# uc-vision/smart-tree

Hardware: AMD Instinct MI355X
Metric: points/sec end-to-end (voxelize->sparse-UNet->skeleton), 1M-pt tree (higher is better)
Workload: dtype f32

## Files before the change

smart_tree_amd/csrc/graph.hip:

```cpp
#include "st_common.h"
#include "st_grid.h"

#define GR_BLOCK 256
static inline unsigned gr_grid(int64_t n) {
    int64_t g = st_div_up(n > 0 ? n : 1, GR_BLOCK);
    return (unsigned)(g < 8192 ? g : 8192);
}
#define GR_LOOP(i, n) for (int64_t i = (int64_t)blockIdx.x * blockDim.x + threadIdx.x; i < (n); i += (int64_t)gridDim.x * blockDim.x)

__global__ void __launch_bounds__(GR_BLOCK) k_medial(const float* xyz, const float* mv, int64_t n, float* medial, float* radius) {
    GR_LOOP(i, n) {
        const float x = mv[3 * i], y = mv[3 * i + 1], z = mv[3 * i + 2];
        medial[3 * i] = xyz[3 * i] + x;
        medial[3 * i + 1] = xyz[3 * i + 1] + y;
        medial[3 * i + 2] = xyz[3 * i + 2] + z;
        float s = x * x;
        float t = y * y;
        s = s + t;
        t = z * z;
        s = s + t;
        radius[i] = sqrtf(s);
    }
}

extern "C" int st_medial_points(const float* xyz, const float* mv, int64_t n, float* medial, float* radius, void* stream_) {
    if (n <= 0) return ST_OK;
    hipLaunchKernelGGL(k_medial, dim3(gr_grid(n)), dim3(GR_BLOCK), 0, (hipStream_t)stream_, xyz, mv, n, medial, radius);
    ST_CHECK_LAUNCH();
    return ST_OK;
}

struct GrRange {
    int64_t i0, i1;
    int64_t a0, a1;
    int64_t nq;
};
__device__ __forceinline__ GrRange gr_range(const void* p0, const void* p1, int64_t n, const int* seg_off, int seg) {
    GrRange r;
    r.i0 = seg_off ? seg_off[seg] : 0;
    r.i1 = seg_off ? seg_off[seg + 1] : n;
    const bool vec = ((((uintptr_t)p0) | ((uintptr_t)p1)) & 15) == 0;
    r.a0 = vec ? st_min((r.i0 + 3) & ~(int64_t)3, r.i1) : r.i1;
    r.a1 = r.a0 + ((r.i1 - r.a0) & ~(int64_t)3);
    r.nq = (r.a1 - r.a0) / 4 * 3;
    return r;
}
__device__ __forceinline__ int64_t gr_edge_point(const GrRange& r, int64_t j) { return j < r.a0 - r.i0 ? r.i0 + j : r.a1 + (j - (r.a0 - r.i0)); }

__global__ void __launch_bounds__(GR_BLOCK) k_bbox(const float* xyz, int64_t n, unsigned* box, const int* seg_off) {
    __shared__ unsigned lo[3], hi[3];
    if (threadIdx.x < 3) { lo[threadIdx.x] = 0xffffffffu; hi[threadIdx.x] = 0u; }
    __syncthreads();
    const int seg = blockIdx.y;
    const GrRange r = gr_range(xyz, nullptr, n, seg_off, seg);
    unsigned lx = 0xffffffffu, ly = 0xffffffffu, lz = 0xffffffffu, hx = 0u, hy = 0u, hz = 0u;
    const float4* v = reinterpret_cast<const float4*>(xyz + 3 * r.a0);
    for (int64_t q = (int64_t)blockIdx.x * blockDim.x + threadIdx.x; q < r.nq; q += (int64_t)gridDim.x * blockDim.x) {
        const float4 f = v[q];
        const int ax = (int)(q % 3);
        const unsigned o0 = st_f2ord(f.x), o1 = st_f2ord(f.y), o2 = st_f2ord(f.z), o3 = st_f2ord(f.w);
        const unsigned a = st_min(o0, o3), b = st_max(o0, o3);
        lx = st_min(lx, ax == 0 ? a : (ax == 1 ? o2 : o1)); hx = st_max(hx, ax == 0 ? b : (ax == 1 ? o2 : o1));
        ly = st_min(ly, ax == 0 ? o1 : (ax == 1 ? a : o2)); hy = st_max(hy, ax == 0 ? o1 : (ax == 1 ? b : o2));
        lz = st_min(lz, ax == 0 ? o2 : (ax == 1 ? o1 : a)); hz = st_max(hz, ax == 0 ? o2 : (ax == 1 ? o1 : b));
    }
    const int64_t ne = (r.a0 - r.i0) + (r.i1 - r.a1);
    for (int64_t j = (int64_t)blockIdx.x * blockDim.x + threadIdx.x; j < ne; j += (int64_t)gridDim.x * blockDim.x) {
        const int64_t i = gr_edge_point(r, j);
        const unsigned ox = st_f2ord(xyz[3 * i]), oy = st_f2ord(xyz[3 * i + 1]), oz = st_f2ord(xyz[3 * i + 2]);
        lx = st_min(lx, ox); hx = st_max(hx, ox); ly = st_min(ly, oy); hy = st_max(hy, oy); lz = st_min(lz, oz); hz = st_max(hz, oz);
    }
    for (int d = 32; d > 0; d >>= 1) {
        lx = st_min(lx, (unsigned)__shfl_xor((int)lx, d)); ly = st_min(ly, (unsigned)__shfl_xor((int)ly, d)); lz = st_min(lz, (unsigned)__shfl_xor((int)lz, d));
        hx = st_max(hx, (unsigned)__shfl_xor((int)hx, d)); hy = st_max(hy, (unsigned)__shfl_xor((int)hy, d)); hz = st_max(hz, (unsigned)__shfl_xor((int)hz, d));
    }
    if ((threadIdx.x & 63) == 0) {
        atomicMin(&lo[0], lx); atomicMin(&lo[1], ly); atomicMin(&lo[2], lz);
        atomicMax(&hi[0], hx); atomicMax(&hi[1], hy); atomicMax(&hi[2], hz);
    }
    __syncthreads();
    if (threadIdx.x < 3 && r.i1 > r.i0) { atomicMin(&box[6 * seg + threadIdx.x], lo[threadIdx.x]); atomicMax(&box[6 * seg + 3 + threadIdx.x], hi[threadIdx.x]); }
}
__global__ void __launch_bounds__(GR_BLOCK) k_centre(const float* xyz, int64_t n, const unsigned* box, float* out, const int* seg_off,
                                                     float* box_out) {
    const int seg = blockIdx.y;
    const GrRange r = gr_range(xyz, out, n, seg_off, seg);
    float shift[3];
    for (int a = 0; a < 3; a++) {
        const float mn = st_ord2f(box[6 * seg + a]), mx = st_ord2f(box[6 * seg + 3 + a]);
        const float half = (mx - mn) / 2.0f;
        const float centre = mn + half;
        shift[a] = -centre + (a == 1 ? half : 0.0f);
        if (box_out && blockIdx.x == 0 && threadIdx.x == 0) {
            box_out[6 * seg + a] = r.i1 > r.i0 ? mn + shift[a] : INFINITY;
            box_out[6 * seg + 3 + a] = r.i1 > r.i0 ? mx + shift[a] : -INFINITY;
        }
    }
    const float4* v = reinterpret_cast<const float4*>(xyz + 3 * r.a0);
    float4* o = reinterpret_cast<float4*>(out + 3 * r.a0);
    for (int64_t q = (int64_t)blockIdx.x * blockDim.x + threadIdx.x; q < r.nq; q += (int64_t)gridDim.x * blockDim.x) {
        float4 f = v[q];
        const int ax = (int)(q % 3);
        const float s0 = ax == 0 ? shift[0] : (ax == 1 ? shift[1] : shift[2]);
        const float s1 = ax == 0 ? shift[1] : (ax == 1 ? shift[2] : shift[0]);
        const float s2 = ax == 0 ? shift[2] : (ax == 1 ? shift[0] : shift[1]);
        f.x = f.x + s0; f.y = f.y + s1; f.z = f.z + s2; f.w = f.w + s0;
        o[q] = f;
    }
    const int64_t ne = (r.a0 - r.i0) + (r.i1 - r.a1);
    for (int64_t j = (int64_t)blockIdx.x * blockDim.x + threadIdx.x; j < ne; j += (int64_t)gridDim.x * blockDim.x) {
        const int64_t i = gr_edge_point(r, j);
        for (int a = 0; a < 3; a++) out[3 * i + a] = xyz[3 * i + a] + shift[a];
    }
}

__global__ void k_box_init(unsigned* box, int nseg) {
    for (int i = threadIdx.x; i < 6 * nseg; i += blockDim.x) box[i] = i % 6 < 3 ? 0xffffffffu : 0u;
}

extern "C" int st_centre_cloud_box_seg(const float* xyz, int64_t n, const int32_t* seg_off, int nseg, float* out, void* ws,
                                       int64_t ws_bytes, void* stream_, float* box_out) {
    hipStream_t stream = (hipStream_t)stream_;
    if (n <= 0) {
        ST_REQUIRE(!box_out, "centre_cloud: no box of an empty array");
        return ST_OK;
    }
    ST_REQUIRE(nseg >= 1 && nseg <= ST_MAX_SEG && (nseg == 1 || seg_off), "centre_cloud: 1 <= clouds per batch <= %d", ST_MAX_SEG);
    if (nseg == 1) seg_off = nullptr;
    StArena a(ws, ws_bytes);
    unsigned* box = a.take<unsigned>(6 * (int64_t)nseg);
    if (!box) { st_set_error("centre_cloud: workspace too small"); return ST_ERR_WORKSPACE; }
    hipLaunchKernelGGL(k_box_init, dim3(1), dim3(64), 0, stream, box, nseg);
    const int64_t per = st_div_up(st_div_up(3 * n, 4), nseg);
    const unsigned gx = (unsigned)st_min64(st_div_up(per > 0 ? per : 1, GR_BLOCK), 2048 / (nseg < 8 ? nseg : 8) + 1);
    hipLaunchKernelGGL(k_bbox, dim3(gx, (unsigned)nseg), dim3(GR_BLOCK), 0, stream, xyz, n, box, seg_off);
    hipLaunchKernelGGL(k_centre, dim3((unsigned)st_min64(st_div_up(per > 0 ? per : 1, GR_BLOCK), 8192), (unsigned)nseg), dim3(GR_BLOCK), 0, stream,
                       xyz, n, (const unsigned*)box, out, seg_off, box_out);
    ST_CHECK_LAUNCH();
    return ST_OK;
}
extern "C" int st_centre_cloud_seg(const float* xyz, int64_t n, const int32_t* seg_off, int nseg, float* out, void* ws,
                                   int64_t ws_bytes, void* stream_) {
    return st_centre_cloud_box_seg(xyz, n, seg_off, nseg, out, ws, ws_bytes, stream_, nullptr);
}
extern "C" int st_centre_cloud(const float* xyz, int64_t n, float* out, void* ws, int64_t ws_bytes, void* stream_) {
    return st_centre_cloud_seg(xyz, n, nullptr, 1, out, ws, ws_bytes, stream_);
}

__global__ void __launch_bounds__(GR_BLOCK) k_edge_count(const int64_t* idx, int64_t n, int K, uint32_t* cnt, const int* seg_off,
                                                         int nseg) {
    GR_LOOP(i, n) {
        const int64_t first = seg_off ? seg_off[st_seg_find(seg_off, nseg, i)] : 0;
        uint32_t c = 0;
        for (int k = 0; k < K; k++) c += idx[i * K + k] > first;
        cnt[i] = c;
    }
}
__global__ void __launch_bounds__(GR_BLOCK) k_edge_emit(const int64_t* idx, const float* dist, int64_t n, int K,
                                                        const uint32_t* off, int64_t* edges, float* w, const int* seg_off,
                                                        int nseg) {
    GR_LOOP(i, n) {
        const int64_t first = seg_off ? seg_off[st_seg_find(seg_off, nseg, i)] : 0;
        uint32_t o = off[i];
        for (int k = 0; k < K; k++) {
            int64_t j = idx[i * K + k];
            if (j > first) { edges[2 * (int64_t)o] = i; edges[2 * (int64_t)o + 1] = j; w[o] = dist[i * K + k]; o++; }
        }
    }
}

extern "C" int64_t st_make_edges_workspace_bytes(int64_t n) {
    StArena a(nullptr, 0);
    a.take<uint32_t>(n + 1);
    a.take<char>(st_scan_ws_bytes(n));
    return a.used;
}

__global__ void __launch_bounds__(GR_BLOCK) k_edge_pad(int64_t* edges, float* w, const uint32_t* total, int64_t cap) {
    for (int64_t e = (int64_t)*total + (int64_t)blockIdx.x * blockDim.x + threadIdx.x; e < cap; e += (int64_t)gridDim.x * blockDim.x) {
        edges[2 * e] = 0;
        edges[2 * e + 1] = 0;
        w[e] = 0.0f;
    }
}

extern "C" int st_make_edges_seg(const int64_t* idx, const float* dist, int64_t n, int K, int64_t* edges, float* w,
                                 int64_t* n_edges_host, const int32_t* seg_off, int nseg, void* ws, int64_t ws_bytes,
                                 void* stream_) {
    hipStream_t stream = (hipStream_t)stream_;
    if (n_edges_host) *n_edges_host = 0;
    if (n <= 0) return ST_OK;
    ST_REQUIRE(nseg >= 1 && nseg <= ST_MAX_SEG && (nseg == 1 || seg_off), "make_edges: 1 <= clouds per batch <= %d", ST_MAX_SEG);
    if (nseg == 1) seg_off = nullptr;
    StArena a(ws, ws_bytes);
    uint32_t* cnt = a.take<uint32_t>(n + 1);
    int64_t sb = st_scan_ws_bytes(n);
    char* sw = a.take<char>(sb);
    if (!cnt || !sw) { st_set_error("make_edges: workspace too small"); return ST_ERR_WORKSPACE; }
    hipLaunchKernelGGL(k_edge_count, dim3(gr_grid(n)), dim3(GR_BLOCK), 0, stream, idx, n, K, cnt, seg_off, nseg);
    ST_TRY(st_exclusive_scan_u32(cnt, cnt, n, cnt + n, sw, sb, stream));
    hipLaunchKernelGGL(k_edge_emit, dim3(gr_grid(n)), dim3(GR_BLOCK), 0, stream, idx, dist, n, K, (const uint32_t*)cnt, edges, w,
                       seg_off, nseg);
    if (!n_edges_host) {
        hipLaunchKernelGGL(k_edge_pad, dim3(64), dim3(GR_BLOCK), 0, stream, edges, w, (const uint32_t*)(cnt + n), n * (int64_t)K);
        ST_CHECK_LAUNCH();
        return ST_OK;
    }
    uint32_t total = 0;
    (void)hipMemcpyAsync(&total, cnt + n, sizeof(uint32_t), hipMemcpyDeviceToHost, stream);
    st_stream_wait(stream);
    ST_CHECK_LAUNCH();
    *n_edges_host = total;
    return ST_OK;
}

extern "C" int st_make_edges(const int64_t* idx, const float* dist, int64_t n, int K, int64_t* edges, float* w,
                             int64_t* n_edges_host, void* ws, int64_t ws_bytes, void* stream_) {
    return st_make_edges_seg(idx, dist, n, K, edges, w, n_edges_host, nullptr, 1, ws, ws_bytes, stream_);
}

struct GrEdges {
    const int64_t* edges;
    const float* w;
    const int64_t* idx;
    const float* dist;
    int K, k_shift;
    const int* first_of;
};
static inline int gr_shift_of(int K) { int sh = 0; while ((1 << sh) < K) sh++; return (1 << sh) == K ? sh : -1; }
__device__ __forceinline__ void gr_edge(const GrEdges& G, int64_t e, int64_t* u, int64_t* v) {
    if (G.idx == nullptr) { *u = G.edges[2 * e]; *v = G.edges[2 * e + 1]; return; }
    const int64_t i = G.k_shift >= 0 ? (e >> G.k_shift) : e / G.K, j = G.idx[e];
    const int64_t first = G.first_of ? G.first_of[i] : 0;
    *u = i;
    *v = j > first ? j : i;
}
__device__ __forceinline__ float gr_edge_weight(const GrEdges& G, int64_t e) { return G.idx ? G.dist[e] : G.w[e]; }

#define CC_MUL 0x9E3779B1u
#define CC_INV 0x0E8B2F51u
__device__ __forceinline__ unsigned cc_key(unsigned x) { return x * CC_MUL; }
__device__ __forceinline__ unsigned cc_idx(unsigned k) { return k * CC_INV; }

__device__ __forceinline__ unsigned cc_find(unsigned* label, unsigned k) {
    unsigned p = __atomic_load_n(&label[cc_idx(k)], __ATOMIC_RELAXED);
    while (p != k) {
        const unsigned gp = __atomic_load_n(&label[cc_idx(p)], __ATOMIC_RELAXED);
        if (gp != p) atomicMin(&label[cc_idx(k)], gp);
        k = p;
        p = gp;
    }
    return k;
}
__global__ void __launch_bounds__(GR_BLOCK) k_cc_init(unsigned* label, int64_t n) { GR_LOOP(i, n) label[i] = cc_key((unsigned)i); }
__global__ void __launch_bounds__(GR_BLOCK) k_cc_hook(GrEdges G, int64_t E, unsigned* label, int sample) {
    GR_LOOP(e, E) {
        if (sample && (((uint32_t)e * 2654435761u) >> 29) != 0u) continue;
        int64_t u64, v64;
        gr_edge(G, e, &u64, &v64);
        const unsigned u = (unsigned)u64, v = (unsigned)v64;
        if (u == v) continue;
        if (!sample) {
            if (label[u] == label[v]) continue;
        }
        unsigned a = cc_find(label, cc_key(u)), b = cc_find(label, cc_key(v));
        while (a != b) {
            if (a < b) { const unsigned t = a; a = b; b = t; }
            const unsigned seen = atomicCAS(&label[cc_idx(a)], a, b);
            if (seen == a) break;
            a = seen;
        }
    }
}
__global__ void __launch_bounds__(GR_BLOCK) k_cc_compress(unsigned* label, int64_t n) {
    GR_LOOP(i, n) { const unsigned r = cc_find(label, cc_key((unsigned)i)); label[i] = r; }
}
__global__ void __launch_bounds__(GR_BLOCK) k_cc_minid_init(unsigned* minid, int64_t n) { GR_LOOP(i, n) minid[i] = 0xffffffffu; }
__global__ void __launch_bounds__(GR_BLOCK) k_cc_minid(const unsigned* label, int64_t n, unsigned* minid) {
    const int lane = threadIdx.x & 63;
    for (int64_t base = (int64_t)blockIdx.x * blockDim.x; base < n; base += (int64_t)gridDim.x * blockDim.x) {
        const int64_t i = base + threadIdx.x;
        const bool valid = i < n;
        const unsigned r = valid ? cc_idx(label[i]) : 0xffffffffu;
        unsigned long long todo = __ballot(valid);
        while (todo) {
            const int leader = __ffsll(todo) - 1;
            const unsigned lr = __shfl(r, leader);
            const unsigned long long same = __ballot(valid && r == lr);
            if (lane == leader) atomicMin(&minid[lr], (unsigned)i);
            todo &= ~same;
        }
    }
}
__global__ void __launch_bounds__(GR_BLOCK) k_cc_relabel(unsigned* label, int64_t n, const unsigned* minid) {
    GR_LOOP(i, n) label[i] = minid[cc_idx(label[i])];
}

extern "C" int64_t st_connected_components_workspace_bytes(int64_t n) { return (n > 0 ? n : 1) * (int64_t)sizeof(unsigned) + 256; }

static int cc_run(GrEdges G, int64_t E, int64_t n, int32_t* labels, void* ws, int64_t ws_bytes, void* stream_);

extern "C" int st_connected_components(const int64_t* edges, int64_t E, int64_t n, int32_t* labels, void* ws,
                                       int64_t ws_bytes, void* stream_) {
    GrEdges G = {edges, nullptr, nullptr, nullptr, 0, -1, nullptr};
    return cc_run(G, E, n, labels, ws, ws_bytes, stream_);
}

extern "C" int st_connected_components_knn(const int64_t* idx, int64_t n, int K, const int32_t* first_of,
                                           int32_t* labels, void* ws, int64_t ws_bytes, void* stream_) {
    ST_REQUIRE(K >= 1, "cc(knn): K must be positive");
    GrEdges G = {nullptr, nullptr, idx, nullptr, K, gr_shift_of(K), first_of};
    return cc_run(G, n * (int64_t)K, n, labels, ws, ws_bytes, stream_);
}

static int cc_run(GrEdges G, int64_t E, int64_t n, int32_t* labels, void* ws, int64_t ws_bytes, void* stream_) {
    hipStream_t stream = (hipStream_t)stream_;
    ST_REQUIRE(n < (1ll << 31), "cc: too many vertices");
    if (n <= 0) return ST_OK;
    StArena ar(ws, ws_bytes);
    unsigned* minid = ar.take<unsigned>(n);
    if (!ar.ok() || !minid) {
        st_set_error("cc: workspace too small (%lld < %lld)", (long long)ws_bytes, (long long)ar.used);
        return ST_ERR_WORKSPACE;
    }
    unsigned* label = (unsigned*)labels;
    hipLaunchKernelGGL(k_cc_init, dim3(gr_grid(n)), dim3(GR_BLOCK), 0, stream, label, n);
    if (E > 0) {
        hipLaunchKernelGGL(k_cc_hook, dim3(gr_grid(E)), dim3(GR_BLOCK), 0, stream, G, E, label, 1);
        hipLaunchKernelGGL(k_cc_compress, dim3(gr_grid(n)), dim3(GR_BLOCK), 0, stream, label, n);
        hipLaunchKernelGGL(k_cc_hook, dim3(gr_grid(E)), dim3(GR_BLOCK), 0, stream, G, E, label, 0);
    }
    hipLaunchKernelGGL(k_cc_compress, dim3(gr_grid(n)), dim3(GR_BLOCK), 0, stream, label, n);
    hipLaunchKernelGGL(k_cc_minid_init, dim3(gr_grid(n)), dim3(GR_BLOCK), 0, stream, minid, n);
    hipLaunchKernelGGL(k_cc_minid, dim3(gr_grid(n)), dim3(GR_BLOCK), 0, stream, (const unsigned*)label, n, minid);
    hipLaunchKernelGGL(k_cc_relabel, dim3(gr_grid(n)), dim3(GR_BLOCK), 0, stream, label, n, (const unsigned*)minid);
    ST_CHECK_LAUNCH();
    return ST_OK;
}

__global__ void __launch_bounds__(GR_BLOCK) k_cl_sizes(const int* label, int64_t n, uint32_t* size) {
    const int lane = threadIdx.x & 63;
    for (int64_t base = (int64_t)blockIdx.x * blockDim.x; base < n; base += (int64_t)gridDim.x * blockDim.x) {
        const int64_t i = base + threadIdx.x;
        const bool valid = i < n;
        const int lab = valid ? label[i] : -1;
        unsigned long long todo = __ballot(valid);
        while (todo) {
            const int leader = __ffsll(todo) - 1;
            const int l = __shfl(lab, leader);
            const unsigned long long same = __ballot(valid && lab == l);
            if (lane == leader) atomicAdd(&size[l], (uint32_t)__popcll(same));
            todo &= ~same;
        }
    }
}
__global__ void __launch_bounds__(GR_BLOCK) k_cl_rootflag(const int* label, const uint32_t* size, int64_t n, uint32_t minv,
                                                          uint32_t* flag, uint32_t* kept) {
    GR_LOOP(i, n) {
        const bool root = label[i] == (int)i && size[i] >= minv;
        flag[i] = root ? 1u : 0u;
        if (root) { atomicAdd(kept, size[i]); atomicMax(kept + 1, size[i]); }
    }
}
__global__ void __launch_bounds__(GR_BLOCK) k_cl_rootlist(const uint32_t* flag_off, const int* label, const uint32_t* size,
                                                          int64_t n, uint32_t minv, uint32_t* key, uint32_t* root) {
    GR_LOOP(i, n) if (label[i] == (int)i && size[i] >= minv) { key[flag_off[i]] = 0xffffffffu - size[i]; root[flag_off[i]] = (uint32_t)i; }
}
__global__ void __launch_bounds__(GR_BLOCK) k_cl_rank(const uint32_t* root_sorted, const uint32_t* size, int64_t C,
                                                      int* rank_of_root, uint32_t* comp_size) {
    GR_LOOP(c, C) { rank_of_root[root_sorted[c]] = (int)c; comp_size[c] = size[root_sorted[c]]; }
}
__global__ void __launch_bounds__(GR_BLOCK) k_cl_segkey(const uint32_t* root_sorted, int64_t C, const int* seg_off, int nseg,
                                                        uint32_t* key) {
    GR_LOOP(c, C) key[c] = (uint32_t)st_seg_find(seg_off, nseg, root_sorted[c]);
}
__global__ void __launch_bounds__(GR_BLOCK) k_cl_segments(const uint32_t* root_sorted, int C, const int* seg_off, int nseg,
                                                          const int32_t* comp_off, int32_t* comp_seg, int32_t* comp_seg_off,
                                                          int32_t* vert_seg_off) {
    for (int b = threadIdx.x; b <= nseg; b += blockDim.x) comp_seg_off[b] = C;
    __syncthreads();
    for (int c = threadIdx.x; c < C; c += blockDim.x) {
        const int s = st_seg_find(seg_off, nseg, root_sorted[c]);
        comp_seg[c] = s;
        const int prev = c > 0 ? st_seg_find(seg_off, nseg, root_sorted[c - 1]) : -1;
        for (int b = prev + 1; b <= s; b++) comp_seg_off[b] = c;
    }
    __syncthreads();
    for (int b = threadIdx.x; b <= nseg; b += blockDim.x) vert_seg_off[b] = comp_off[comp_seg_off[b]];
}
__global__ void __launch_bounds__(GR_BLOCK) k_cl_vflag(const int* label, const int* rank_of_root, int64_t n, uint32_t* flag) {
    GR_LOOP(i, n) flag[i] = rank_of_root[label[i]] >= 0 ? 1u : 0u;
}
__global__ void __launch_bounds__(GR_BLOCK) k_cl_vlist(const uint32_t* flag_off, const int* label, const int* rank_of_root,
                                                       int64_t n, uint32_t* vkey, uint32_t* vid) {
    GR_LOOP(i, n) {
        int r = rank_of_root[label[i]];
        if (r >= 0) { vkey[flag_off[i]] = (uint32_t)r; vid[flag_off[i]] = (uint32_t)i; }
    }
}
__global__ void __launch_bounds__(GR_BLOCK) k_cl_newid(const uint32_t* vid_sorted, int64_t m, int* new_id, int32_t* vert_order) {
    GR_LOOP(p, m) { new_id[vid_sorted[p]] = (int)p; vert_order[p] = (int32_t)vid_sorted[p]; }
}
__global__ void __launch_bounds__(GR_BLOCK) k_fill_i32(int* p, int64_t n, int v) { GR_LOOP(i, n) p[i] = v; }

extern "C" int64_t st_component_layout_workspace_bytes(int64_t n) {
    StArena a(nullptr, 0);
    a.take<uint32_t>(n + 2);
    a.take<uint32_t>(n + 1);
    a.take<uint32_t>(n);
    a.take<uint32_t>(n);
    a.take<int>(n);
    a.take<char>(st_sort_ws_bytes(n) > st_scan_ws_bytes(n + 1) ? st_sort_ws_bytes(n) : st_scan_ws_bytes(n + 1));
    return a.used;
}

extern "C" int st_component_layout_seg(const int32_t* labels, int64_t n, int min_vertices, const int32_t* seg_off, int nseg,
                                       int32_t* comp_size, int32_t* comp_off, int32_t* vert_order, int32_t* new_id,
                                       int32_t* comp_seg, int32_t* comp_seg_off, int32_t* vert_seg_off,
                                       int64_t* n_comp_host, int64_t* n_kept_host, void* ws, int64_t ws_bytes, void* stream_,
                                       int64_t* max_comp_host ) {
    hipStream_t stream = (hipStream_t)stream_;
    *n_comp_host = 0;
    *n_kept_host = 0;
    if (max_comp_host) *max_comp_host = 0;
    ST_REQUIRE(nseg >= 1 && nseg <= ST_MAX_SEG, "component_layout: 1 <= clouds per batch <= %d", ST_MAX_SEG);
    ST_REQUIRE(nseg == 1 || (seg_off && comp_seg && comp_seg_off && vert_seg_off), "component_layout: a batch needs seg_off and the per-cloud outputs");
    if (n <= 0) {
        if (nseg > 1) { (void)hipMemsetAsync(comp_seg_off, 0, (nseg + 1) * sizeof(int32_t), stream); (void)hipMemsetAsync(vert_seg_off, 0, (nseg + 1) * sizeof(int32_t), stream); }
        return ST_OK;
    }
    StArena a(ws, ws_bytes);
    uint32_t* size = a.take<uint32_t>(n + 2);
    uint32_t* flag = a.take<uint32_t>(n + 1);
    uint32_t* key = a.take<uint32_t>(n);
    uint32_t* val = a.take<uint32_t>(n);
    int* rank_of_root = a.take<int>(n);
    int64_t sb = st_sort_ws_bytes(n) > st_scan_ws_bytes(n + 1) ? st_sort_ws_bytes(n) : st_scan_ws_bytes(n + 1);
    char* sw = a.take<char>(sb);
    if (!a.ok() || !sw) { st_set_error("component_layout: workspace too small"); return ST_ERR_WORKSPACE; }
    const unsigned g = gr_grid(n);
    uint32_t minv = min_vertices > 0 ? (uint32_t)min_vertices : 0u;
    (void)hipMemsetAsync(size, 0, (n + 2) * sizeof(uint32_t), stream);
    hipLaunchKernelGGL(k_cl_sizes, dim3(g), dim3(GR_BLOCK), 0, stream, labels, n, size);
    hipLaunchKernelGGL(k_cl_rootflag, dim3(g), dim3(GR_BLOCK), 0, stream, labels, (const uint32_t*)size, n, minv, flag, size + n);
    ST_TRY(st_exclusive_scan_u32(flag, flag, n, flag + n, sw, sb, stream));
    uint32_t C = 0, mk[2] = {0, 0};
    (void)hipMemcpyAsync(&C, flag + n, sizeof(uint32_t), hipMemcpyDeviceToHost, stream);
    (void)hipMemcpyAsync(mk, size + n, 2 * sizeof(uint32_t), hipMemcpyDeviceToHost, stream);
    st_stream_wait(stream);
    const uint32_t m = mk[0];
    if (max_comp_host) *max_comp_host = mk[1];
    ST_CHECK_LAUNCH();
    hipLaunchKernelGGL(k_fill_i32, dim3(g), dim3(GR_BLOCK), 0, stream, new_id, n, -1);
    if (C == 0) {
        (void)hipMemsetAsync(comp_off, 0, sizeof(int32_t), stream);
        if (nseg > 1) { (void)hipMemsetAsync(comp_seg_off, 0, (nseg + 1) * sizeof(int32_t), stream); (void)hipMemsetAsync(vert_seg_off, 0, (nseg + 1) * sizeof(int32_t), stream); }
        ST_CHECK_LAUNCH();
        return ST_OK;
    }
    hipLaunchKernelGGL(k_cl_rootlist, dim3(g), dim3(GR_BLOCK), 0, stream, (const uint32_t*)flag, labels, (const uint32_t*)size, n,
                       minv, key, val);
    ST_TRY(st_radix_sort_pairs_u32(key, val, C, 32, sw, sb, stream));
    if (nseg > 1) {
        int sbits = 1;
        while ((1 << sbits) < nseg) sbits++;
        hipLaunchKernelGGL(k_cl_segkey, dim3(gr_grid(C)), dim3(GR_BLOCK), 0, stream, (const uint32_t*)val, (int64_t)C, seg_off, nseg, key);
        ST_TRY(st_radix_sort_pairs_u32(key, val, C, sbits, sw, sb, stream));
    }
    hipLaunchKernelGGL(k_fill_i32, dim3(g), dim3(GR_BLOCK), 0, stream, rank_of_root, n, -1);
    hipLaunchKernelGGL(k_cl_rank, dim3(gr_grid(C)), dim3(GR_BLOCK), 0, stream, (const uint32_t*)val, (const uint32_t*)size,
                       (int64_t)C, rank_of_root, (uint32_t*)comp_size);
    ST_TRY(st_exclusive_scan_u32((const uint32_t*)comp_size, (uint32_t*)comp_off, C, (uint32_t*)comp_off + C, sw, sb, stream));
    if (nseg > 1)
        hipLaunchKernelGGL(k_cl_segments, dim3(1), dim3(GR_BLOCK), 0, stream, (const uint32_t*)val, (int)C, seg_off, nseg,
                           (const int32_t*)comp_off, comp_seg, comp_seg_off, vert_seg_off);
    hipLaunchKernelGGL(k_cl_vflag, dim3(g), dim3(GR_BLOCK), 0, stream, labels, (const int*)rank_of_root, n, flag);
    ST_TRY(st_exclusive_scan_u32(flag, flag, n, flag + n, sw, sb, stream));
    hipLaunchKernelGGL(k_cl_vlist, dim3(g), dim3(GR_BLOCK), 0, stream, (const uint32_t*)flag, labels, (const int*)rank_of_root, n,
                       key, val);
    int bits = 1;
    while ((1u << bits) < C && bits < 32) bits++;
    ST_TRY(st_radix_sort_pairs_u32(key, val, m, bits, sw, sb, stream));
    hipLaunchKernelGGL(k_cl_newid, dim3(gr_grid(m)), dim3(GR_BLOCK), 0, stream, (const uint32_t*)val, (int64_t)m, new_id,
                       vert_order);
    ST_CHECK_LAUNCH();
    *n_comp_host = C;
    *n_kept_host = m;
    return ST_OK;
}

extern "C" int st_component_layout(const int32_t* labels, int64_t n, int min_vertices, int32_t* comp_size, int32_t* comp_off,
                                   int32_t* vert_order, int32_t* new_id, int64_t* n_comp_host, int64_t* n_kept_host,
                                   void* ws, int64_t ws_bytes, void* stream_) {
    return st_component_layout_seg(labels, n, min_vertices, nullptr, 1, comp_size, comp_off, vert_order, new_id, nullptr, nullptr,
                                   nullptr, n_comp_host, n_kept_host, ws, ws_bytes, stream_, nullptr);
}

__device__ __forceinline__ uint32_t gr_run_add(uint32_t* ctr, int key) {
    const int lane = threadIdx.x & 63;
    const int prev = __shfl_up(key, 1);
    const bool head = key >= 0 && (lane == 0 || prev != key);
    const unsigned long long heads = __ballot(head), active = __ballot(key >= 0);
    const unsigned long long upto = heads & (~0ull >> (63 - lane));
    const int h = 63 - __clzll((long long)(upto | 1ull));
    const unsigned long long stop = (heads | ~active) & ~(~0ull >> (63 - h));
    const int end = stop ? __ffsll((long long)stop) - 1 : 64;
    uint32_t base = 0;
    if (head) base = atomicAdd(&ctr[key], (uint32_t)(end - lane));
    base = __shfl(base, h);
    return base + (uint32_t)(lane - h);
}

__device__ __forceinline__ void csr_edge_ends(const GrEdges& G, int64_t E, const int* new_id, int64_t e, int* a, int* b) {
    *a = -1; *b = -1;
    if (e >= E) return;
    int64_t u, v;
    gr_edge(G, e, &u, &v);
    if (u == v) return;
    const int x = new_id[u], y = new_id[v];
    if (x < 0 || y < 0) return;
    *a = x; *b = y;
}

__global__ void __launch_bounds__(GR_BLOCK) k_csr_count(GrEdges G, int64_t E, const int* new_id, uint32_t* deg) {
    const int lane = threadIdx.x & 63;
    for (int64_t base = (int64_t)blockIdx.x * blockDim.x + (threadIdx.x - lane); base < E; base += (int64_t)gridDim.x * blockDim.x) {
        int a, b;
        csr_edge_ends(G, E, new_id, base + lane, &a, &b);
        gr_run_add(deg, a);
        if (b >= 0) atomicAdd(&deg[b], 1u);
    }
}
__global__ void __launch_bounds__(GR_BLOCK) k_csr_fill(GrEdges G, int64_t E, const int* new_id,
                                                       uint32_t* cursor, uint32_t* col, float* wgt) {
    const int lane = threadIdx.x & 63;
    for (int64_t base = (int64_t)blockIdx.x * blockDim.x + (threadIdx.x - lane); base < E; base += (int64_t)gridDim.x * blockDim.x) {
        int a, b;
        csr_edge_ends(G, E, new_id, base + lane, &a, &b);
        const uint32_t pa = gr_run_add(cursor, a);
        if (a < 0) continue;
        const float we = gr_edge_weight(G, base + lane);
        col[pa] = (uint32_t)b; wgt[pa] = we;
        const uint32_t pb = atomicAdd(&cursor[b], 1u);
        col[pb] = (uint32_t)a; wgt[pb] = we;
    }
}

#define CSRK_MUTUAL 0x40000000
struct __attribute__((aligned(16))) GrI64x2 { int64_t x, y; };
struct __attribute__((aligned(16))) GrI32x4 { int32_t x, y, z, w; };
__global__ void __launch_bounds__(GR_BLOCK) k_csrk_pack(const int64_t* __restrict__ idx, int64_t E, int32_t* __restrict__ idx32) {
    GR_LOOP(e, E) idx32[e] = (int32_t)idx[e];
}
template <int K, bool PACKED>
__global__ void __launch_bounds__(GR_BLOCK) k_csrk_count(const int64_t* __restrict__ idx, const int32_t* __restrict__ idx32, int64_t n,
                                                         const int* __restrict__ first_of, const int* __restrict__ new_id, uint32_t* deg,
                                                         uint32_t* fwdc, int32_t* __restrict__ tgt) {
    const int64_t E = n * K;
    const int lane = threadIdx.x & 63;
    for (int64_t base = (int64_t)blockIdx.x * blockDim.x + (threadIdx.x - lane); base < E; base += (int64_t)gridDim.x * blockDim.x) {
        const int64_t e = base + lane;
        const int64_t i = e / K;
        int x = -1, y = -1;
        bool mutual = false;
        if (e < E) {
            x = new_id[i];
            const int64_t j = PACKED ? (int64_t)idx32[e] : idx[e], first = first_of ? first_of[i] : 0;
            if (x >= 0 && j > first && j != i) {
                y = new_id[j];
                if (y >= 0 && i > first) {
                    const int64_t* row = idx + j * K;
                    if (PACKED && K % 4 == 0) {
                        const int32_t* row32 = idx32 + j * K;
                        const int32_t i32 = (int32_t)i;
#pragma unroll
                        for (int k = 0; k < K; k += 4) {
                            const GrI32x4 r = *reinterpret_cast<const GrI32x4*>(row32 + k);
                            mutual = mutual || r.x == i32 || r.y == i32 || r.z == i32 || r.w == i32;
                        }
                    } else if (PACKED) {
                        for (int k = 0; k < K; k++) mutual = mutual || (int64_t)idx32[j * K + k] == i;
                    } else if (K % 2 == 0) {
#pragma unroll
                        for (int k = 0; k < K; k += 2) {
                            const GrI64x2 r = *reinterpret_cast<const GrI64x2*>(row + k);
                            mutual = mutual || r.x == i || r.y == i;
                        }
                    } else {
                        for (int k = 0; k < K; k++) mutual = mutual || row[k] == i;
                    }
                }
            }
        }
        const bool fwd = y >= 0;
        const unsigned long long fb = __ballot(fwd);
        if (e < E) tgt[e] = fwd ? (y | (mutual ? CSRK_MUTUAL : 0)) : -1;
        if (fwd && !mutual) atomicAdd(&deg[y], 1u);
        if ((lane % K) == 0 && x >= 0) {
            const unsigned cnt = (unsigned)__popcll(K == 64 ? fb : (fb >> lane) & ((1ull << (K & 63)) - 1ull));
            fwdc[x] = cnt;
            if (cnt) atomicAdd(&deg[x], cnt);
        }
    }
}
template <int K>
__global__ void __launch_bounds__(GR_BLOCK) k_csrk_fill(const int64_t n, const float* __restrict__ dist, const int* __restrict__ new_id,
                                                        const int32_t* __restrict__ tgt, const uint32_t* __restrict__ row_off,
                                                        uint32_t* cursor, uint32_t* __restrict__ col, float* __restrict__ wgt) {
    const int64_t E = n * K;
    const int lane = threadIdx.x & 63;
    for (int64_t base = (int64_t)blockIdx.x * blockDim.x + (threadIdx.x - lane); base < E; base += (int64_t)gridDim.x * blockDim.x) {
        const int64_t e = base + lane;
        const int32_t t = e < E ? tgt[e] : -1;
        const bool fwd = t >= 0;
        const unsigned long long fb = __ballot(fwd);
        if (!fwd) continue;
        const int x = new_id[e / K], y = t & ~CSRK_MUTUAL;
        const float we = dist[e];
        const int k = lane % K;
        const unsigned long long mine = K == 64 ? fb : (fb >> (lane - k)) & ((1ull << (K & 63)) - 1ull);
        const uint32_t pa = row_off[x] + (uint32_t)__popcll(mine & ((1ull << k) - 1ull));
        col[pa] = (uint32_t)y; wgt[pa] = we;
        if (!(t & CSRK_MUTUAL)) {
            const uint32_t pb = atomicAdd(&cursor[y], 1u);
            col[pb] = (uint32_t)x; wgt[pb] = we;
        }
    }
}
__global__ void __launch_bounds__(GR_BLOCK) k_csrk_cursor(const uint32_t* __restrict__ row_off, const uint32_t* __restrict__ fwdc, int64_t m,
                                                          uint32_t* __restrict__ cursor) {
    GR_LOOP(v, m) cursor[v] = row_off[v] + fwdc[v];
}

extern "C" int64_t st_component_csr_workspace_bytes(int64_t m) {
    StArena a(nullptr, 0);
    a.take<uint32_t>(m + 1);
    a.take<char>(st_scan_ws_bytes(m + 1));
    return a.used;
}
extern "C" int64_t st_component_csr_knn_workspace_bytes(int64_t m, int64_t n, int K) {
    StArena a(nullptr, 0);
    a.take<uint32_t>(m + 1);
    a.take<char>(st_scan_ws_bytes(m + 1));
    a.take<uint32_t>(m + 1);
    a.take<int32_t>(n * (int64_t)(K > 0 ? K : 1));
    a.take<int32_t>(n * (int64_t)(K > 0 ? K : 1));
    return a.used;
}

static int csr_run(GrEdges G, int64_t E, const int32_t* new_id, int64_t m, uint32_t* row_off, uint32_t* col, float* wgt, void* ws,
                   int64_t ws_bytes, void* stream_);

extern "C" int st_component_csr(const int64_t* edges, const float* w, int64_t E, const int32_t* new_id, int64_t m,
                                uint32_t* row_off, uint32_t* col, float* wgt, void* ws, int64_t ws_bytes, void* stream_) {
    GrEdges G = {edges, w, nullptr, nullptr, 0, -1, nullptr};
    return csr_run(G, E, new_id, m, row_off, col, wgt, ws, ws_bytes, stream_);
}

template <int K>
static void csrk_launch(const int64_t* idx, const float* dist, int64_t n, const int32_t* first_of, const int32_t* new_id, int64_t m,
                        uint32_t* row_off, uint32_t* col, float* wgt, uint32_t* cursor, uint32_t* fwdc, int32_t* tgt, int32_t* idx32,
                        char* sw, int64_t sb, hipStream_t stream, int* rc) {
    const int64_t E = n * K;
    (void)hipMemsetAsync(row_off, 0, (m + 1) * sizeof(uint32_t), stream);
    if (idx32) {
        hipLaunchKernelGGL(k_csrk_pack, dim3(gr_grid(E)), dim3(GR_BLOCK), 0, stream, idx, E, idx32);
        hipLaunchKernelGGL((k_csrk_count<K, true>), dim3(gr_grid(E)), dim3(GR_BLOCK), 0, stream, idx, (const int32_t*)idx32, n, first_of,
                           new_id, row_off, fwdc, tgt);
    } else {
        hipLaunchKernelGGL((k_csrk_count<K, false>), dim3(gr_grid(E)), dim3(GR_BLOCK), 0, stream, idx, (const int32_t*)nullptr, n, first_of,
                           new_id, row_off, fwdc, tgt);
    }
    *rc = st_exclusive_scan_u32(row_off, row_off, m + 1, nullptr, sw, sb, stream);
    if (*rc != ST_OK) return;
    hipLaunchKernelGGL(k_csrk_cursor, dim3(gr_grid(m)), dim3(GR_BLOCK), 0, stream, (const uint32_t*)row_off, (const uint32_t*)fwdc, m, cursor);
    hipLaunchKernelGGL((k_csrk_fill<K>), dim3(gr_grid(E)), dim3(GR_BLOCK), 0, stream, n, dist, new_id, (const int32_t*)tgt,
                       (const uint32_t*)row_off, cursor, col, wgt);
}
extern "C" int st_component_csr_knn(const int64_t* idx, const float* dist, int64_t n, int K, const int32_t* first_of,
                                    const int32_t* new_id, int64_t m, uint32_t* row_off, uint32_t* col, float* wgt, void* ws,
                                    int64_t ws_bytes, void* stream_) {
    ST_REQUIRE(K >= 1, "csr(knn): K must be positive");
    hipStream_t stream = (hipStream_t)stream_;
    if (m > 0 && n > 0 && gr_shift_of(K) >= 0 && K <= 64 && ws_bytes >= st_component_csr_knn_workspace_bytes(m, n, K)) {
        ST_REQUIRE(m < CSRK_MUTUAL, "csr(knn): too many vertices");
        StArena a(ws, ws_bytes);
        uint32_t* cursor = a.take<uint32_t>(m + 1);
        const int64_t sb = st_scan_ws_bytes(m + 1);
        char* sw = a.take<char>(sb);
        uint32_t* fwdc = a.take<uint32_t>(m + 1);
        int32_t* tgt = a.take<int32_t>(n * (int64_t)K);
        int32_t* idx32 = a.take<int32_t>(n * (int64_t)K);
        if (!cursor || !sw || !fwdc || !tgt || !idx32) { st_set_error("component_csr(knn): workspace too small"); return ST_ERR_WORKSPACE; }
        if (n >= (1ll << 31)) idx32 = nullptr;
        int rc = ST_OK;
#define CSRK_CASE(K_) case K_: csrk_launch<K_>(idx, dist, n, first_of, new_id, m, row_off, col, wgt, cursor, fwdc, tgt, idx32, sw, sb, stream, &rc); break;
        switch (K) { CSRK_CASE(1) CSRK_CASE(2) CSRK_CASE(4) CSRK_CASE(8) CSRK_CASE(16) CSRK_CASE(32) CSRK_CASE(64) }
#undef CSRK_CASE
        if (rc != ST_OK) return rc;
        ST_CHECK_LAUNCH();
        return ST_OK;
    }
    GrEdges G = {nullptr, nullptr, idx, dist, K, gr_shift_of(K), first_of};
    return csr_run(G, n * (int64_t)K, new_id, m, row_off, col, wgt, ws, ws_bytes, stream_);
}

static int csr_run(GrEdges G, int64_t E, const int32_t* new_id, int64_t m, uint32_t* row_off, uint32_t* col, float* wgt, void* ws,
                   int64_t ws_bytes, void* stream_) {
    hipStream_t stream = (hipStream_t)stream_;
    if (m <= 0) return ST_OK;
    StArena a(ws, ws_bytes);
    uint32_t* cursor = a.take<uint32_t>(m + 1);
    int64_t sb = st_scan_ws_bytes(m + 1);
    char* sw = a.take<char>(sb);
    if (!cursor || !sw) { st_set_error("component_csr: workspace too small"); return ST_ERR_WORKSPACE; }
    (void)hipMemsetAsync(row_off, 0, (m + 1) * sizeof(uint32_t), stream);
    if (E > 0) hipLaunchKernelGGL(k_csr_count, dim3(gr_grid(E)), dim3(GR_BLOCK), 0, stream, G, E, new_id, row_off);
    ST_TRY(st_exclusive_scan_u32(row_off, row_off, m + 1, nullptr, sw, sb, stream));
    (void)hipMemcpyAsync(cursor, row_off, (m + 1) * sizeof(uint32_t), hipMemcpyDeviceToDevice, stream);
    if (E > 0) hipLaunchKernelGGL(k_csr_fill, dim3(gr_grid(E)), dim3(GR_BLOCK), 0, stream, G, E, new_id, cursor, col, wgt);
    ST_CHECK_LAUNCH();
    return ST_OK;
}
```

Baseline: 1.008 billion.

## Fuse component layout for small component counts into single-block bitonic kernel

Computes the per-vertex kept flag alongside the root flag and scans both before the host sync. The root list and the fills are launched before the sync as well. When the component count fits in shared memory (at most 4096), one single-block kernel replaces the radix sort(s), rank, scan and segment kernels: it does a bitonic sort on a combined segment and size key, then scans offsets and writes the segment outputs. This cuts kernel launches and sort passes in the middle of the pipeline, at the cost of an extra n-sized scan and workspace buffer, and a serial single-block path.

Result: slower. 992.8 million (-1.5%).

```diff
diff --git a/smart_tree_amd/csrc/graph.hip b/smart_tree_amd/csrc/graph.hip
--- a/smart_tree_amd/csrc/graph.hip
+++ b/smart_tree_amd/csrc/graph.hip
@@ -355,11 +355,14 @@
     }
 }
 __global__ void __launch_bounds__(GR_BLOCK) k_cl_rootflag(const int* label, const uint32_t* size, int64_t n, uint32_t minv,
-                                                          uint32_t* flag, uint32_t* kept) {
+                                                          uint32_t* flag, uint32_t* vflag, uint32_t* kept) {
     GR_LOOP(i, n) {
-        const bool root = label[i] == (int)i && size[i] >= minv;
+        const int lab = label[i];
+        const uint32_t sz = size[lab];
+        const bool root = lab == (int)i && sz >= minv;
         flag[i] = root ? 1u : 0u;
-        if (root) { atomicAdd(kept, size[i]); atomicMax(kept + 1, size[i]); }
+        vflag[i] = sz >= minv && label[lab] == lab ? 1u : 0u;
+        if (root) { atomicAdd(kept, sz); atomicMax(kept + 1, sz); }
     }
 }
 __global__ void __launch_bounds__(GR_BLOCK) k_cl_rootlist(const uint32_t* flag_off, const int* label, const uint32_t* size,
@@ -388,8 +391,71 @@
     __syncthreads();
     for (int b = threadIdx.x; b <= nseg; b += blockDim.x) vert_seg_off[b] = comp_off[comp_seg_off[b]];
 }
-__global__ void __launch_bounds__(GR_BLOCK) k_cl_vflag(const int* label, const int* rank_of_root, int64_t n, uint32_t* flag) {
-    GR_LOOP(i, n) flag[i] = rank_of_root[label[i]] >= 0 ? 1u : 0u;
+#define CL_SMALL_CAP 4096
+__global__ void __launch_bounds__(GR_BLOCK) k_cl_small(const uint32_t* key, const uint32_t* root, int C, const int* seg_off, int nseg,
+                                                       int* rank_of_root, uint32_t* comp_size, uint32_t* comp_off, int32_t* comp_seg,
+                                                       int32_t* comp_seg_off, int32_t* vert_seg_off) {
+    __shared__ uint64_t s_key[CL_SMALL_CAP];
+    __shared__ uint32_t s_root[CL_SMALL_CAP];
+    __shared__ uint32_t s_part[GR_BLOCK];
+    __shared__ int32_t s_seg_off[ST_MAX_SEG + 1];
+    const int tid = threadIdx.x;
+    int P = 1;
+    while (P < C) P <<= 1;
+    for (int c = tid; c < P; c += GR_BLOCK) {
+        const bool in = c < C;
+        const uint32_t r = in ? root[c] : 0xffffffffu;
+        s_root[c] = r;
+        s_key[c] = in ? ((uint64_t)st_seg_find(seg_off, nseg, r) << 32) | key[c] : ~0ull;
+    }
+    __syncthreads();
+    for (int k = 2; k <= P; k <<= 1)
+        for (int j = k >> 1; j > 0; j >>= 1) {
+            for (int t = tid; t < (P >> 1); t += GR_BLOCK) {
+                const int lo = ((t & ~(j - 1)) << 1) | (t & (j - 1)), hi = lo | j;
+                const uint64_t ka = s_key[lo], kb = s_key[hi];
+                const uint32_t ra = s_root[lo], rb = s_root[hi];
+                const bool gt = ka > kb || (ka == kb && ra > rb);
+                if (gt == ((lo & k) == 0)) { s_key[lo] = kb; s_key[hi] = ka; s_root[lo] = rb; s_root[hi] = ra; }
+            }
+            __syncthreads();
+        }
+    const int per = P > GR_BLOCK ? P / GR_BLOCK : 1;
+    const int c0 = tid * per, c1 = c0 + per < C ? c0 + per : C;
+    uint32_t sum = 0;
+    for (int c = c0; c < c1; c++) sum += 0xffffffffu - (uint32_t)s_key[c];
+    s_part[tid] = sum;
+    __syncthreads();
+    for (int d = 1; d < GR_BLOCK; d <<= 1) {
+        const uint32_t add = tid >= d ? s_part[tid - d] : 0u;
+        __syncthreads();
+        s_part[tid] += add;
+        __syncthreads();
+    }
+    uint32_t off = s_part[tid] - sum;
+    for (int c = c0; c < c1; c++) {
+        const uint32_t sz = 0xffffffffu - (uint32_t)s_key[c];
+        rank_of_root[s_root[c]] = c;
+        comp_size[c] = sz;
+        comp_off[c] = off;
+        s_key[c] = (s_key[c] & 0xffffffff00000000ull) | off;
+        off += sz;
+    }
+    if (tid == GR_BLOCK - 1) comp_off[C] = s_part[GR_BLOCK - 1];
+    if (nseg <= 1) return;
+    for (int b = tid; b <= nseg; b += GR_BLOCK) s_seg_off[b] = C;
+    __syncthreads();
+    for (int c = tid; c < C; c += GR_BLOCK) {
+        const int s = (int)(s_key[c] >> 32), prev = c > 0 ? (int)(s_key[c - 1] >> 32) : -1;
+        comp_seg[c] = s;
+        for (int b = prev + 1; b <= s; b++) s_seg_off[b] = c;
+    }
+    __syncthreads();
+    for (int b = tid; b <= nseg; b += GR_BLOCK) {
+        const int c = s_seg_off[b];
+        comp_seg_off[b] = c;
+        vert_seg_off[b] = c < C ? (int32_t)(uint32_t)s_key[c] : (int32_t)s_part[GR_BLOCK - 1];
+    }
 }
 __global__ void __launch_bounds__(GR_BLOCK) k_cl_vlist(const uint32_t* flag_off, const int* label, const int* rank_of_root,
                                                        int64_t n, uint32_t* vkey, uint32_t* vid) {
@@ -406,6 +472,7 @@
 extern "C" int64_t st_component_layout_workspace_bytes(int64_t n) {
     StArena a(nullptr, 0);
     a.take<uint32_t>(n + 2);
+    a.take<uint32_t>(n + 1);
     a.take<uint32_t>(n + 1);
     a.take<uint32_t>(n);
     a.take<uint32_t>(n);
@@ -432,6 +499,7 @@
     StArena a(ws, ws_bytes);
     uint32_t* size = a.take<uint32_t>(n + 2);
     uint32_t* flag = a.take<uint32_t>(n + 1);
+    uint32_t* vflag = a.take<uint32_t>(n + 1);
     uint32_t* key = a.take<uint32_t>(n);
     uint32_t* val = a.take<uint32_t>(n);
     int* rank_of_root = a.take<int>(n);
@@ -442,8 +510,13 @@
     uint32_t minv = min_vertices > 0 ? (uint32_t)min_vertices : 0u;
     (void)hipMemsetAsync(size, 0, (n + 2) * sizeof(uint32_t), stream);
     hipLaunchKernelGGL(k_cl_sizes, dim3(g), dim3(GR_BLOCK), 0, stream, labels, n, size);
-    hipLaunchKernelGGL(k_cl_rootflag, dim3(g), dim3(GR_BLOCK), 0, stream, labels, (const uint32_t*)size, n, minv, flag, size + n);
+    hipLaunchKernelGGL(k_cl_rootflag, dim3(g), dim3(GR_BLOCK), 0, stream, labels, (const uint32_t*)size, n, minv, flag, vflag, size + n);
     ST_TRY(st_exclusive_scan_u32(flag, flag, n, flag + n, sw, sb, stream));
+    ST_TRY(st_exclusive_scan_u32(vflag, vflag, n, vflag + n, sw, sb, stream));
+    hipLaunchKernelGGL(k_cl_rootlist, dim3(g), dim3(GR_BLOCK), 0, stream, (const uint32_t*)flag, labels, (const uint32_t*)size, n,
+                       minv, key, val);
+    hipLaunchKernelGGL(k_fill_i32, dim3(g), dim3(GR_BLOCK), 0, stream, new_id, n, -1);
+    hipLaunchKernelGGL(k_fill_i32, dim3(g), dim3(GR_BLOCK), 0, stream, rank_of_root, n, -1);
     uint32_t C = 0, mk[2] = {0, 0};
     (void)hipMemcpyAsync(&C, flag + n, sizeof(uint32_t), hipMemcpyDeviceToHost, stream);
     (void)hipMemcpyAsync(mk, size + n, 2 * sizeof(uint32_t), hipMemcpyDeviceToHost, stream);
@@ -451,32 +524,31 @@
     const uint32_t m = mk[0];
     if (max_comp_host) *max_comp_host = mk[1];
     ST_CHECK_LAUNCH();
-    hipLaunchKernelGGL(k_fill_i32, dim3(g), dim3(GR_BLOCK), 0, stream, new_id, n, -1);
     if (C == 0) {
         (void)hipMemsetAsync(comp_off, 0, sizeof(int32_t), stream);
         if (nseg > 1) { (void)hipMemsetAsync(comp_seg_off, 0, (nseg + 1) * sizeof(int32_t), stream); (void)hipMemsetAsync(vert_seg_off, 0, (nseg + 1) * sizeof(int32_t), stream); }
         ST_CHECK_LAUNCH();
         return ST_OK;
     }
-    hipLaunchKernelGGL(k_cl_rootlist, dim3(g), dim3(GR_BLOCK), 0, stream, (const uint32_t*)flag, labels, (const uint32_t*)size, n,
-                       minv, key, val);
-    ST_TRY(st_radix_sort_pairs_u32(key, val, C, 32, sw, sb, stream));
-    if (nseg > 1) {
-        int sbits = 1;
-        while ((1 << sbits) < nseg) sbits++;
-        hipLaunchKernelGGL(k_cl_segkey, dim3(gr_grid(C)), dim3(GR_BLOCK), 0, stream, (const uint32_t*)val, (int64_t)C, seg_off, nseg, key);
-        ST_TRY(st_radix_sort_pairs_u32(key, val, C, sbits, sw, sb, stream));
-    }
-    hipLaunchKernelGGL(k_fill_i32, dim3(g), dim3(GR_BLOCK), 0, stream, rank_of_root, n, -1);
-    hipLaunchKernelGGL(k_cl_rank, dim3(gr_grid(C)), dim3(GR_BLOCK), 0, stream, (const uint32_t*)val, (const uint32_t*)size,
-                       (int64_t)C, rank_of_root, (uint32_t*)comp_size);
-    ST_TRY(st_exclusive_scan_u32((const uint32_t*)comp_size, (uint32_t*)comp_off, C, (uint32_t*)comp_off + C, sw, sb, stream));
-    if (nseg > 1)
-        hipLaunchKernelGGL(k_cl_segments, dim3(1), dim3(GR_BLOCK), 0, stream, (const uint32_t*)val, (int)C, seg_off, nseg,
-                           (const int32_t*)comp_off, comp_seg, comp_seg_off, vert_seg_off);
-    hipLaunchKernelGGL(k_cl_vflag, dim3(g), dim3(GR_BLOCK), 0, stream, labels, (const int*)rank_of_root, n, flag);
-    ST_TRY(st_exclusive_scan_u32(flag, flag, n, flag + n, sw, sb, stream));
-    hipLaunchKernelGGL(k_cl_vlist, dim3(g), dim3(GR_BLOCK), 0, stream, (const uint32_t*)flag, labels, (const int*)rank_of_root, n,
+    if (C <= CL_SMALL_CAP) {
+        hipLaunchKernelGGL(k_cl_small, dim3(1), dim3(GR_BLOCK), 0, stream, (const uint32_t*)key, (const uint32_t*)val, (int)C, seg_off,
+                           nseg, rank_of_root, (uint32_t*)comp_size, (uint32_t*)comp_off, comp_seg, comp_seg_off, vert_seg_off);
+    } else {
+        ST_TRY(st_radix_sort_pairs_u32(key, val, C, 32, sw, sb, stream));
+        if (nseg > 1) {
+            int sbits = 1;
+            while ((1 << sbits) < nseg) sbits++;
+            hipLaunchKernelGGL(k_cl_segkey, dim3(gr_grid(C)), dim3(GR_BLOCK), 0, stream, (const uint32_t*)val, (int64_t)C, seg_off, nseg, key);
+            ST_TRY(st_radix_sort_pairs_u32(key, val, C, sbits, sw, sb, stream));
+        }
+        hipLaunchKernelGGL(k_cl_rank, dim3(gr_grid(C)), dim3(GR_BLOCK), 0, stream, (const uint32_t*)val, (const uint32_t*)size,
+                           (int64_t)C, rank_of_root, (uint32_t*)comp_size);
+        ST_TRY(st_exclusive_scan_u32((const uint32_t*)comp_size, (uint32_t*)comp_off, C, (uint32_t*)comp_off + C, sw, sb, stream));
+        if (nseg > 1)
+            hipLaunchKernelGGL(k_cl_segments, dim3(1), dim3(GR_BLOCK), 0, stream, (const uint32_t*)val, (int)C, seg_off, nseg,
+                               (const int32_t*)comp_off, comp_seg, comp_seg_off, vert_seg_off);
+    }
+    hipLaunchKernelGGL(k_cl_vlist, dim3(g), dim3(GR_BLOCK), 0, stream, (const uint32_t*)vflag, labels, (const int*)rank_of_root, n,
                        key, val);
     int bits = 1;
     while ((1u << bits) < C && bits < 32) bits++;
```
